# rainerzufalldererste/limg

Measured on AMD Instinct MI355X. Metric: encode Mpixels/s, 8K RGBA (limg_encode3d_test-equivalent: all 11 planes stored), higher is better.
Workload: dtype u8/i32 integer stage + f32 float stage (bit-exact vs the reference's strict SSE build)

## Files before the change

limg_amd/csrc/limg_hip_kernels.hip:

```cpp
#include "limg_hip_phase_e.h"
#include "limg_hip_lookback.h"

namespace limg_hip
{
  namespace
  {
    constexpr int kPrioE = 2;


    template <int CH, bool PERSIST, class P>
    __device__ __forceinline__ void finish_block(const P &p, const EStrip g, const uint32_t sb, const uint32_t bx, const BlkF *blkE, const uint32_t shift[3], const uint32_t fA,
                                                 const uint32_t fB, const uint32_t fC, const bool active, const uint32_t o, uint8_t *park, uint8_t *stage, uint32_t &waveCalls)
    {
      const uint32_t calls = (((shift[0] & 7u) + 7u) >> 3) + (((shift[1] & 7u) + 7u) >> 3) + (((shift[2] & 7u) + 7u) >> 3);
      waveCalls += calls;
      if (p.stripWords)
      {
        uint32_t words = 0;
#pragma unroll
        for (int k = 0; k < 3; k++)
        {
          const uint32_t sk = shift[k];
          if (sk < 8u) words += 8u - sk;
          else if (CH == 4 && sgpr((int)blkE->rec[8 * k + 3]) != sgpr((int)blkE->rec[8 * k + 7])) words += 8u;
// ... 37 lines not shown

    template <bool PERSIST, class P, class IO>
    __device__ __forceinline__ void park_or_store_factors(const P &p, const IO &io, const EStrip g, uint8_t *park, uint8_t *stage)
    {
      if (PERSIST)
        for (int i = g.tid; i < 384; i += kThreads) reinterpret_cast<uint4 *>(park + kParkFac)[i] = *reinterpret_cast<const uint4 *>(stage + (i >> 4) * kFacRow + (i & 15) * 16);
      else if (p.storePlanes) copy_factor_planes<true>(p, io, stage, g.x0, g.y0, g.stripW, g.ry, g.tid);
    }

    template <int CH, bool PERSIST, bool FAST, bool PREFIT, bool ACC, bool NOSEL, class P, class LIM, class IO>
    __device__ __forceinline__ void fit_search_strip(const P &p, const LIM &lim, const IO &io, const uint32_t id, const uint32_t local, const uint32_t rowBase, const uint32_t head0, uint8_t *lds,
                                                     uint8_t *park, const int tid)
    {
      constexpr LdsLayout LL = lds_layout<PREFIT>();
      EStrip g;
      g.tid = tid; g.lane = tid & 63; g.wave = tid >> 6;
      g.strip = local % p.stripsX; g.by = local / p.stripsX; g.byS = rowBase + g.by;
      g.x0 = g.strip * (kStripBlocks * kBlock); g.y0 = g.by * kBlock;
      g.stripW = min(p.sizeX - g.x0, (uint32_t)(kStripBlocks * kBlock)); g.ry = min(p.sizeY - g.y0, (uint32_t)kBlock);
      g.pix = reinterpret_cast<uint32_t *>(lds + kLdsStrip); g.V = reinterpret_cast<float *>(lds + LL.v); g.blk = reinterpret_cast<BlkF *>(lds + LL.blk);
      g.calls = reinterpret_cast<uint32_t *>(lds + LL.calls); g.trialc = reinterpret_cast<int *>(lds + LL.trialc);
      const int lane = g.lane;

      uint32_t recVal[2] = { 0u, 0u };
      if (PREFIT) request_prefit_records(p, g, recVal);
      stage_strip_pixels(p, io, g);
      __syncthreads();
      if (PREFIT) take_prefit_records<PERSIST>(p, g, recVal, park);
      else
      {
      const unsigned short *s_rsq = d_rsqrt_x86_tab;
      const int lane = g.lane, wave = g.wave;
      const uint32_t strip = g.strip, by = g.by, byS = g.byS;
      float *V = g.V + wave * kBatch * kVDw;
      BlkF *blk = g.blk + wave * kBlocksPerWave;
      auto geom = [&](int b, uint32_t &rx, uint32_t &n) -> bool { return block_geom(p, g, wave * kBlocksPerWave + b, rx, n); };

#pragma unroll 1
      for (int h = 0; h < kBlocksPerWave / kBatch; h++)
      {
      uint32_t px8[kBatch];
      V4 est8[kBatch];
      BlkF *const blkh = blk + h * kBatch;

#pragma unroll
      for (int i = 0; i < kBatch; i++)
      {
        const int b = h * kBatch + i;
        uint32_t rx, n;
        px8[i] = 0;
        est8[i].a = float2_t{ 0.0f, 0.0f }; est8[i].b = float2_t{ 0.0f, 0.0f };
        if (!geom(b, rx, n))
        {
// ... 161 lines not shown
        const int b = lane >> 3, j = lane & 7;
        const uint32_t flags = blk[b].flags;
        uint32_t big = 0;
#pragma unroll
        for (int r = 0; r < 3; r++)
        {
          const int kc = j + 8 * r, k = kc >> 2, c = kc & 3;
          const float *dir = r == 0 ? blk[b].dirA : (r == 1 ? blk[b].dirB : blk[b].dirC);
          const int sl = slot_of(c);
          float m = blk[b].mm[k], dv = dir[sl];
          const bool dead = (r == 2 && (flags & kZeroC)) || (r >= 1 && (flags & kZeroB)) || (flags & kZeroA);
          if (dead) { m = 0.0f; dv = 0.0f; }
          float val = m * dv;
          if (r == 0) val = blk[b].avg[sl] + val;
          int q = cvt_rne(val);
          if ((CH == 3 && c == 3) || !(flags & kValid)) q = 0;
          big |= (q > p.recordLimit || q < -p.recordLimit) ? 1u : 0u;
          blk[b].rec[kc] = (int16_t)q;
        }
        big |= (uint32_t)dpp<0xB1, 0xF>(0, (int)big);
        big |= (uint32_t)dpp<0x4E, 0xF>(0, (int)big);
        big |= (uint32_t)dpp<0x141, 0xF>(0, (int)big);
        if (j == 0 && big) blk[b].flags = flags | kBig;
      }
      wave_lds_fence();
      {
#pragma unroll
        for (int r = 0; r < 2; r++)
        {
          const int b = r * 4 + (lane >> 4), w = lane & 15;
          const uint32_t sb = wave * kBlocksPerWave + b, bx = strip * kStripBlocks + sb;
          const uint32_t val = w < 4 ? __float_as_uint(blk[b].avg[slot_of(w)]) : reinterpret_cast<const uint32_t *>(blk[b].rec)[w - 4];
          if (bx < p.blocksX && (!PERSIST || p.compactOut)) reinterpret_cast<uint32_t *>(p.records + (size_t)byS * p.blocksX + bx)[w] = val;
          if (PERSIST && w >= 4) reinterpret_cast<uint32_t *>(park + kParkRec)[sb * 12 + (w - 4)] = val;
        }
      }
    
      }
      if (!PERSIST && p.fitOnly) return;
      phase_e_view<CH, FAST, PREFIT>(g);
      uint32_t *s_queue = g.calls + 4;
      if (tid == 0) *s_queue = 0;
      __syncthreads();

      uint8_t *stage = reinterpret_cast<uint8_t *>(g.V);
      uint32_t waveCalls = 0;

      auto grab = [&]() -> uint32_t { uint32_t v = 0; if (lane == 0) v = atomicAdd(s_queue, 1u); return (uint32_t)sgpr((int)v); };
      uint32_t sbNext = grab();
#pragma unroll 1
      for (;;)
      {
        const uint32_t sb = sbNext;
        if (sb >= (uint32_t)kStripBlocks) break;
        uint32_t qv = 0;
        if (lane == 0) qv = atomicAdd(s_queue, 1u);
        uint32_t rx, n, lx, ly;
        if (!block_geom(p, g, sb, rx, n)) { sbNext = (uint32_t)sgpr((int)qv); continue; }
        const BlkF *const blkE = g.blk + sb;
        const bool active = (uint32_t)lane < n;
        const uint32_t px = block_pixel(g, sb, rx, n, lx, ly);
        uint32_t fA, fB, fC, shift[3] = { 0, 0, 0 };
        pixel_factors<CH, FAST>(reinterpret_cast<const BlkE *>(blkE), px, fA, fB, fC);
        if (p.forced[0] >= 0) { shift[0] = (uint32_t)p.forced[0]; shift[1] = (uint32_t)p.forced[1]; shift[2] = (uint32_t)p.forced[2]; }
        else if (lim.crushBits)
        {
// ... 79 lines not shown
        if (is_head(e)) { sum = 0; flag = 1; }
        sum += p.stripCalls[e];
      }
      s_sum[t] = sum; s_flag[t] = flag;
      __syncthreads();
      for (uint32_t off = 1; off < 1024; off <<= 1)
      {
        uint32_t vs = s_sum[t], vf = s_flag[t];
        if (t >= off && !vf) { vs += s_sum[t - off]; vf = s_flag[t - off]; }
        __syncthreads();
        s_sum[t] = vs; s_flag[t] = vf;
        __syncthreads();
      }
      uint32_t run = (t == 0) ? 0u : s_sum[t - 1];
      for (uint32_t e = begin; e < end; e++)
      {
        if (is_head(e)) run = 0;
        p.stripBase[e] = run;
        run += p.stripCalls[e];
      }
      if (p.chainCallsOut && end == total && begin < end) *p.chainCallsOut = run;
    }

    static_assert(kPhaseFBytes + kStripBlocks * 48 <= kLdsTotal - kLdsStrip - 16, "the F step's LDS overlays the E step's");

    template <int CH, bool PERSIST, class P, class IO>
    __device__ __forceinline__ void dither_store_strip(const P &p, const IO &io, const uint32_t id, const uint32_t local, const uint32_t rowBase, const uint32_t head0, uint8_t *fbase,
                                                       const uint8_t *park, const int tid)
    {
      int16_t *s_rec = reinterpret_cast<int16_t *>(fbase + kPhaseFBytes);
      const int lane = tid & 63, wave = tid >> 6;
      const uint32_t strip = local % p.stripsX, by = local / p.stripsX;
      const uint32_t byS = rowBase + by;
      const uint32_t x0 = strip * (kStripBlocks * kBlock), y0 = by * kBlock;
      const uint32_t stripW = min(p.sizeX - x0, (uint32_t)(kStripBlocks * kBlock));
      const uint32_t ry = min(p.sizeY - y0, (uint32_t)kBlock);
      const uint32_t nBlocks = min(p.blocksX - strip * kStripBlocks, (uint32_t)kStripBlocks);
      const StripLds L = carve_phase_f(fbase, s_rec, 24);

      if (PERSIST)
      {
        static_assert(kStripBlocks * 12 * 4 == 96 * 16, "record copy");
#pragma unroll 1
        for (int i = tid; i < 384; i += kThreads) *reinterpret_cast<uint4 *>(L.fac + (i >> 4) * kFacRow + (i & 15) * 16) = reinterpret_cast<const uint4 *>(park + kParkFac)[i];
        if (tid < 96) reinterpret_cast<uint4 *>(s_rec)[tid] = reinterpret_cast<const uint4 *>(park + kParkRec)[tid];
        if (tid < kStripBlocks) L.shift[tid] = (uint32_t)tid < nBlocks ? reinterpret_cast<const uint32_t *>(park + kParkShift)[tid] : 0u;
      }
      else
      {
        copy_factor_planes<false>(p, io, L.fac, x0, y0, stripW, ry, tid);
        for (int i = tid; i < kStripBlocks * 12; i += kThreads)
        {
          const int sb = i / 12, w = i - sb * 12;
          uint32_t v = 0;
          if ((uint32_t)sb < nBlocks) v = reinterpret_cast<const uint32_t *>(p.records + (size_t)byS * p.blocksX + strip * kStripBlocks + sb)[4 + w];
          reinterpret_cast<uint32_t *>(s_rec + sb * 24)[w] = v;
        }
        if (tid < kStripBlocks) L.shift[tid] = (uint32_t)tid < nBlocks ? p.shifts[(size_t)byS * p.blocksX + strip * kStripBlocks + tid] : 0u;
      }
      __syncthreads();
      phase_f_prepare<CH>(L, lane, wave, p.recordLimit);
      wave_lds_fence();
      const bool rowsPath = PERSIST || (p.sizeX % kBlock == 0 && ry == (uint32_t)kBlock);
      if (p.fullPlanes) phase_f_store_const(p, io, L, x0, y0, ry, lane, wave, rowsPath ? 1u : 3u);
      if (wave == 0)
      {
        uint32_t base;
        if (PERSIST)
        {
          const uint32_t headId = head0 + chain_head_row(p.chainCount, p.chainRows, by) * p.stripsX;
          const uint32_t w = lane < kStripBlocks ? L.shift[lane] : 0u;
          const uint32_t agg = wave_sum(w >> 24);
          const unsigned long long own = desc_load(p.desc + id);
          if ((uint32_t)(own >> 32) == kDescInclusive) base = (uint32_t)sgpr((int)((uint32_t)own == kBasePoison ? kBasePoison : (uint32_t)own - agg));
          else
          {
            base = lookback_base(p, id, headId, agg, lane);
            if (lane == 0 && publishes(p, id)) desc_store(p.desc + id, kDescInclusive, base == kBasePoison ? kBasePoison : base + agg);
          }
#ifdef LIMG_HIP_TEST_HOOKS
          if (id == p.testBaseErrStrip) base += 1u;
#endif
        }
        else
        {
          base = p.stripBase[id];
          if (p.chainBase) base += (uint32_t)*p.chainBase;
        }
        phase_f_first_calls(L, base, lane);
      }
      __syncthreads();
      if (PERSIST && L.first[0] == kBasePoison) return;
      if (rowsPath) phase_f_rows<CH>(p, io, L, strip, x0, y0, lane, wave, [&]() { if (p.fullPlanes) phase_f_store_const(p, io, L, x0, y0, ry, lane, wave, 2u); });
      else phase_f_pixels<CH>(p, io, L, strip, x0, y0, ry, lane, wave, tid);
    }

    template <int CH, bool FAST, bool PREFIT, bool ACC>
    __global__ __launch_bounds__(kThreads) void k_fit_search(const EncodeParams p)
    {
      __shared__ __attribute__((aligned(16))) uint8_t s_lds[lds_layout<PREFIT>().total];
      if (red_select_dead(p.maxPixel32)) fit_search_strip<CH, false, FAST, PREFIT, ACC, true>(p, p, p.io, blockIdx.x, blockIdx.x, 0u, 0u, s_lds, nullptr, (int)threadIdx.x);
      else fit_search_strip<CH, false, FAST, PREFIT, ACC, false>(p, p, p.io, blockIdx.x, blockIdx.x, 0u, 0u, s_lds, nullptr, (int)threadIdx.x);
    }

    template <int CH>
    __global__ __launch_bounds__(kThreads) void k_dither_store(const EncodeParams p)
    {
      __shared__ __attribute__((aligned(16))) uint8_t s_lds[kPhaseFBytes + kStripBlocks * 48];
      if (p.chainBase && *p.chainBase == ~0ull) return;
      dither_store_strip<CH, false>(p, p.io, blockIdx.x, blockIdx.x, 0u, 0u, s_lds, nullptr, (int)threadIdx.x);
    }

    template <int CH, bool FAST, bool PREFIT, bool ACC>
    __global__ __launch_bounds__(kThreads, PREFIT ? 6 : 5) void k_encode_persistent(const EncodeParams p)
    {
      __shared__ __attribute__((aligned(16))) uint8_t s_lds[lds_layout<PREFIT>().total];
      __shared__ uint32_t s_ticket;
      typedef const __attribute__((address_space(4))) EncodeParams KernArgs;
      typedef const __attribute__((address_space(4))) ImageIO KernIO;
      auto io_of = [](KernArgs *a, uint32_t img) -> KernIO * { return a->batchCount > 1 ? (KernIO *)a->batch + img : &a->io; };
#define LIMG_LOOP_LIMITS(a, img) (*(a))
#define LIMG_LOOP_STRIPS (p.imageStrips * p.batchCount)
#define LIMG_LOOP_FIND_IMAGE(a, t, img) if ((a)->batchCount > 1) img = (t) / (a)->imageStrips;
#define LIMG_LOOP_HEAD0(a, img) ((img) * (a)->imageStrips)
#define LIMG_LOOP_ROWBASE(a, img) ((img) * (a)->blocksY)
#define LIMG_LOOP_VIEW(a, img) (a)
      if (red_select_dead(p.maxPixel32))
      {
        constexpr bool NOSEL = true;
#include "limg_hip_persistent_loop.inc"
      }
// ... 190 lines not shown
```

limg_amd/csrc/limg_hip_phase_e.h:

```cpp
#ifndef LIMG_HIP_PHASE_E_H
#define LIMG_HIP_PHASE_E_H

#include "limg_hip_search.h"
#include "limg_hip_phase_f.h"
#include "limg_hip_float_pixel.h"

namespace limg_hip
{
  namespace
  {
    constexpr int kLdsStrip = 0, kLdsV = kLdsStrip + 8 * kRowDw * 4, kLdsVBytes = kWaves * kBatch * kVDw * 4;
    constexpr int kLdsBlk = kLdsV + kLdsVBytes, kLdsCalls = kLdsBlk + kStripBlocks * 192, kLdsTotal = kLdsCalls + 32;
    static_assert(kLdsTotal <= 32768 - 16, "5 workgroups per CU");
    struct LdsLayout { int v, blk, calls, trialc, total; };
    constexpr int kTrialConstDw = 20;
    template <bool PREFIT> __device__ __host__ constexpr LdsLayout lds_layout()
    {
      if (!PREFIT) return LdsLayout{ kLdsV, kLdsBlk, kLdsCalls, kLdsV, kLdsTotal };
      const int v = kLdsStrip + 8 * kRowDw * 4, blk = v + kFacBytes, calls = blk + kStripBlocks * 192, tc = calls + 32, e = tc + kStripBlocks * kTrialConstDw * 4;
      const int f = kLdsStrip + kPhaseFBytes + kStripBlocks * 48 + 16;
      return LdsLayout{ v, blk, calls, tc, e > f ? e : f };
    }
    static_assert(lds_layout<true>().total <= 163840 / 6, "6 workgroups per CU with the float stage in its own kernel");


    constexpr int kParkFac = 0, kParkRec = 6144, kParkShift = 6144 + 1536, kParkBytes = 8192;


    template <class P>
    __device__ __forceinline__ void request_prefit_records(const P &p, const EStrip g, uint32_t recVal[2])
    {
#pragma unroll
      for (int r = 0; r < 2; r++)
      {
        const int b = r * 4 + (g.lane >> 4), w = g.lane & 15;
        const uint32_t bx = g.strip * kStripBlocks + g.wave * kBlocksPerWave + b;
        if (bx < p.blocksX) recVal[r] = w >= 4 ? reinterpret_cast<const uint32_t *>(p.records + (size_t)g.byS * p.blocksX + bx)[w]
                                               : reinterpret_cast<const uint32_t *>(p.invN)[((size_t)g.byS * p.blocksX + bx) * 4 + w];
      }
    }

    template <class P, class IO>
    __device__ __forceinline__ void stage_strip_pixels(const P &p, const IO &io, const EStrip g)
    {
      const int tid = g.tid;
      if (p.vecIn)
      {
#pragma unroll
        for (int pass = 0; pass < 2; pass++)
        {
          const uint32_t row = pass * 4 + (tid >> 6), col = (tid & 63) * 4;
          if (row < g.ry && col < g.stripW)
          {
            const uint4 v = *reinterpret_cast<const uint4 *>(io.in + (size_t)(g.y0 + row) * p.sizeX + g.x0 + col);
            *reinterpret_cast<uint4 *>(&g.pix[row * kRowDw + col]) = v;
          }
        }
      }
      else
      {
        for (uint32_t i = tid; i < 8 * 256; i += kThreads)
        {
          const uint32_t row = i >> 8, col = i & 255;
          if (row < g.ry && col < g.stripW) g.pix[row * kRowDw + col] = io.in[(size_t)(g.y0 + row) * p.sizeX + g.x0 + col];
        }
      }
    }

    template <bool PERSIST, class P>
    __device__ __forceinline__ void take_prefit_records(const P &p, const EStrip g, const uint32_t recVal[2], uint8_t *park)
    {
      BlkF *blk = g.blk + g.wave * kBlocksPerWave;
#pragma unroll
      for (int r = 0; r < 2; r++)
      {
        const int b = r * 4 + (g.lane >> 4), w = g.lane & 15;
        const uint32_t sb = g.wave * kBlocksPerWave + b, bx = g.strip * kStripBlocks + sb;
        const uint32_t val = recVal[r];
        if (w < 3) reinterpret_cast<BlkE *>(&blk[b])->invN[w] = __uint_as_float(val);
        if (w >= 4)
        {
          reinterpret_cast<uint32_t *>(blk[b].rec)[w - 4] = val;
          if (PERSIST) reinterpret_cast<uint32_t *>(park + kParkRec)[sb * 12 + (w - 4)] = val;
        }
        const int lo = (int)(int16_t)(val & 0xFFFFu), hi = (int)(int16_t)(val >> 16);
        uint32_t big = (w >= 4 && (lo > p.recordLimit || lo < -p.recordLimit || hi > p.recordLimit || hi < -p.recordLimit)) ? 1u : 0u;
        big |= (uint32_t)dpp<0xB1, 0xF>(0, (int)big);
        big |= (uint32_t)dpp<0x4E, 0xF>(0, (int)big);
        big |= (uint32_t)dpp<0x141, 0xF>(0, (int)big);
        big |= (uint32_t)dpp<0x140, 0xF>(0, (int)big);
        if (w == 0) { blk[b].flags = (bx < p.blocksX ? kValid : 0u) | (big ? kBig : 0u); blk[b].n = bx < p.blocksX ? 64u : 0u; }
      }
      wave_lds_fence();
    }

    template <int CH, bool FAST, bool PREFIT>
    __device__ __forceinline__ void phase_e_view(const EStrip g)
    {
      const int lane = g.lane;
      BlkF *blk = g.blk + g.wave * kBlocksPerWave;
      float nrm[2], off[2], invn[2];
#pragma unroll
      for (int r = 0; r < 2; r++)
      {
        const int idx = min(r * 64 + lane, 95);
        const int b = idx / 12, fc = idx - b * 12, f = fc >> 2, c = fc & 3;
        const int lo = blk[b].rec[f * 8 + c], hi = blk[b].rec[f * 8 + 4 + c];
        nrm[r] = (float)(hi - lo); off[r] = (float)lo;
        if (PREFIT) { invn[r] = 0.0f; continue; }
        const float sq = nrm[r] * nrm[r];
        const float s0 = __int_as_float(dpp<0x00, 0xF>(0, __float_as_int(sq))), s1 = __int_as_float(dpp<0x55, 0xF>(0, __float_as_int(sq)));
        const float s2 = __int_as_float(dpp<0xAA, 0xF>(0, __float_as_int(sq))), s3 = __int_as_float(dpp<0xFF, 0xF>(0, __float_as_int(sq)));
        float s = ((0.0f + s0) + s1) + s2;
        if (CH == 4) s = s + s3;
        const bool nz = (s0 != 0.0f) || (s1 != 0.0f) || (s2 != 0.0f) || (CH == 4 && s3 != 0.0f);
        invn[r] = nz ? (FAST ? __builtin_amdgcn_rcpf(s) : 1.0f / s) : 0.0f;
      }
      wave_lds_fence();
#pragma unroll
      for (int r = 0; r < 2; r++)
      {
        const int idx = r * 64 + lane;
        if (idx < 96)
        {
          const int b = idx / 12, fc = idx - b * 12, f = fc >> 2, c = fc & 3;
          BlkE *e = reinterpret_cast<BlkE *>(&blk[b]);
          e->nrm[f][slot_of(c)] = nrm[r]; e->off[f][slot_of(c)] = off[r];
          if (!PREFIT && c == 0) e->invN[f] = invn[r];
          if (PREFIT && c < 3)
          {
            int *tc = g.trialc + (g.wave * kBlocksPerWave + b) * kTrialConstDw;
            tc[f * 3 + c] = -(int)nrm[r];
            tc[9 + f * 3 + c] = term_const(f, c, (int)off[r]);
          }
        }
      }
    }

    template <int CH, bool FAST>
    __device__ __forceinline__ void pixel_factors(const BlkE *be, const uint32_t px, uint32_t &fA, uint32_t &fB, uint32_t &fC)
    {
      const V4 pv = px_to_v4(px);
      const V4 nA = ld4(be->nrm[0]), mnA = ld4(be->off[0]);
      const float fa = dp4<CH, FAST>(pv - mnA, nA) * be->invN[0];
      fA = cvt_u8_rne_sat(255.0f * fa);
      const V4 nB = ld4(be->nrm[1]), ofB = ld4(be->off[1]);
      V4 est = mnA + nA * fa;
      const float fb = dp4<CH, FAST>((pv - est) - ofB, nB) * be->invN[1];
      fB = cvt_u8_rne_sat(255.0f * fb);
      const V4 nC = ld4(be->nrm[2]), ofC = ld4(be->off[2]);
      est = est + nB * fb;
      const float fc = dp4<CH, FAST>((pv - est) - ofC, nC) * be->invN[2];
      fC = cvt_u8_rne_sat(255.0f * fc);
    }
  }
}

// ... 2 lines not shown
```

limg_amd/csrc/limg_hip_phase_f.h:

```cpp
#ifndef LIMG_HIP_PHASE_F_H
#define LIMG_HIP_PHASE_F_H

#include "limg_hip_search.h"
#include <type_traits>

namespace limg_hip
{
  namespace
  {
    constexpr int kFacRow = 320, kFacPlane = 8 * kFacRow, kFacBytes = 3 * kFacPlane;

    template <bool TO_PLANES, class P, class IO>
    __device__ __forceinline__ void copy_factor_planes(const P &p, const IO &io, uint8_t *fac, const uint32_t x0, const uint32_t y0, const uint32_t stripW, const uint32_t ry, const int tid)
    {
      uint8_t *planes[3] = { io.info.pFactorsA, io.info.pFactorsB, io.info.pFactorsC };
      auto piece = [&](auto *g, auto *l) { if (TO_PLANES) *g = *l; else *l = *g; };
      if (p.vecFactors)
        for (int i = tid; i < 384; i += kThreads)
        {
          const int pl = i >> 7, row = (i & 127) >> 4, col = (i & 15) * 16;
          if ((uint32_t)row < ry && (uint32_t)col < stripW)
            piece(reinterpret_cast<uint4 *>(planes[pl] + (size_t)(y0 + row) * p.sizeX + x0 + col), reinterpret_cast<uint4 *>(fac + pl * kFacPlane + row * kFacRow + col));
        }
      else
        for (int i = tid; i < 3 * 2048; i += kThreads)
        {
          const int pl = i >> 11, row = (i & 2047) >> 8, col = i & 255;
          if ((uint32_t)row < ry && (uint32_t)col < stripW) piece(planes[pl] + (size_t)(y0 + row) * p.sizeX + x0 + col, fac + pl * kFacPlane + row * kFacRow + col);
        }
    }

    struct StripLds
    {
      uint8_t *fac;
      uint32_t *dec;
      uint8_t *out;
      uint32_t *cst;
      int32_t *nm;
      uint32_t *shift;
      uint32_t *first;
      uint32_t *flags;
      const int16_t *rec;
      int recStride;
    };
    constexpr int kPhaseFBytes = kFacBytes + 8192 + 3584 + 3072 + 128 + 128 + 128;

    __device__ __forceinline__ StripLds carve_phase_f(uint8_t *base, const int16_t *rec, int recStride)
    {
      StripLds L;
      L.fac = base;
      L.dec = reinterpret_cast<uint32_t *>(base + kFacBytes);
      L.out = base;
      L.cst = reinterpret_cast<uint32_t *>(base + kFacBytes + 8192);
      L.nm = reinterpret_cast<int32_t *>(base + kFacBytes + 8192 + 3584);
      L.shift = reinterpret_cast<uint32_t *>(base + kFacBytes + 8192 + 3584 + 3072);
      L.first = L.shift + 32;
      L.flags = L.shift + 64;
      L.rec = rec; L.recStride = recStride;
      return L;
    }

    __device__ __forceinline__ constexpr int decode_bias(int factor, int c) { return c < 2 ? (term_bias(factor) << 8) : 0; }

    template <int CH>
    __device__ __forceinline__ void phase_f_prepare(const StripLds &L, int lane, int wave, int recordLimit)
    {
      if (lane < 56)
      {
        const int b = lane / 7, k = lane - b * 7, sb = wave * kBlocksPerWave + b;
        const int16_t *rec = L.rec + sb * L.recStride;
        uint32_t v;
        if (k == 0)
        {
          const uint32_t w = L.shift[sb];
          const uint32_t pat[3] = { (w & 0xFF), ((w >> 8) & 0xFF), ((w >> 16) & 0xFF) };
          const uint32_t pa = pat[0] == 8 ? 0xFFu : pat[0] * 0x22u, pb = pat[1] == 8 ? 0xFFu : pat[1] * 0x22u, pc = pat[2] == 8 ? 0xFFu : pat[2] * 0x22u;
          v = 0xFF000000u | (pa << 16) | (pb << 8) | pc;
        }
        else
        {
          v = 0;
#pragma unroll
          for (int c = 0; c < CH; c++)
          {
            int q = rec[(k - 1) * 4 + c] + (k >= 3 ? 0x80 : 0);
            q = q < 0 ? 0 : (q > 255 ? 255 : q);
            v |= (uint32_t)q << (8 * c);
          }
          if (CH == 3) v |= 0xFF000000u;
        }
        reinterpret_cast<uint4 *>(L.cst)[k * kStripBlocks + sb] = make_uint4(v, v, v, v);
      }
      if (lane < kBlocksPerWave)
      {
        const int sb = wave * kBlocksPerWave + lane;
        const int16_t *rec = L.rec + sb * L.recStride;
        uint32_t fl;
        if (CH == 3) fl = 255u << 8;
        else
        {
          const bool varies = rec[7] != rec[3] || rec[15] != rec[11] || rec[23] != rec[19];
          int a = rec[3] + rec[11] + rec[19];
          a = a < 0 ? 0 : (a > 255 ? 255 : a);
          fl = varies ? 2u : ((uint32_t)a << 8);
        }
        L.flags[sb] = fl;
      }
      wave_lds_fence();
#pragma unroll
      for (int r = 0; r < 2; r++)
      {
        const int idx = r * 64 + lane;
        if (idx < 96)
        {
          const int b = idx / 12, fc = idx - b * 12, f = fc >> 2, c = fc & 3, sb = wave * kBlocksPerWave + b;
          const int16_t *rec = L.rec + sb * L.recStride;
          const uint32_t sh = (L.shift[sb] >> (8 * f)) & 0xFF;
          const int lo = rec[f * 8 + c], hi = rec[f * 8 + 4 + c];
          if ((uint32_t)(lo + recordLimit) > 2u * (uint32_t)recordLimit || (uint32_t)(hi + recordLimit) > 2u * (uint32_t)recordLimit) atomicOr(&L.flags[sb], 1u);
          int n = hi - lo, m = lo;
          if (c < 3)
          {
            if (sh > 7) { n = 0; if (f > 0) m = 0; }
          }
          else if (CH == 3) { n = 0; m = 0xFFFF; }
          int *dst = L.nm + sb * 24;
          dst[f * 4 + c] = n;
          dst[12 + f * 4 + c] = (int)(((uint32_t)m << 8) + 128u + (uint32_t)(c < 2 ? (f == 2 ? 0x200000 : 0x300000) : 0));
        }
      }
    }

    typedef uint32_t u32x4_t __attribute__((ext_vector_type(4)));
    typedef uint32_t u32x2_t __attribute__((ext_vector_type(2)));
    __device__ __forceinline__ void plane_store16(void *dst, const uint4 &v)
    {
      __builtin_nontemporal_store(u32x4_t{ v.x, v.y, v.z, v.w }, reinterpret_cast<u32x4_t *>(dst));
    }
    __device__ __forceinline__ void plane_store8(void *dst, const uint2 &v)
    {
      __builtin_nontemporal_store(u32x2_t{ v.x, v.y }, reinterpret_cast<u32x2_t *>(dst));
    }

    template <class P, class IO>
    __device__ __forceinline__ void phase_f_store_const(const P &p, const IO &io, const StripLds &L, uint32_t x0, uint32_t y0, uint32_t ry, int lane, int wave, const uint32_t halves = 3u)
    {
      const uint32_t wx0 = x0 + wave * 64;
      if (wx0 >= p.sizeX) return;
      const uint32_t ww = min(p.sizeX - wx0, 64u);
      uint32_t *planes[7] = { io.info.pShiftABCX, io.info.pColAMin, io.info.pColAMax, io.info.pColBMin, io.info.pColBMax, io.info.pColCMin, io.info.pColCMax };
      if (p.vecPlanes)
      {
        const uint32_t col = ((uint32_t)lane & 15u) * 4u, rsub = (uint32_t)lane >> 4;
// ... 87 lines not shown
      const uint32_t j = (uint32_t)lane & 7u, r = (uint32_t)lane >> 3;
      const uint32_t sb = (uint32_t)wave * kBlocksPerWave + j, bx = strip * kStripBlocks + sb;
      const bool valid = bx < p.blocksX;
      const uint32_t w = L.shift[sb], fl = L.flags[sb];
      uint32_t call = L.first[sb];
      const size_t g = (size_t)(y0 + r) * p.sizeX + x0 + sb * kBlock;
      uint2 nz[3];
#pragma unroll
      for (int k = 0; k < 3; k++)
      {
        const uint32_t s = (w >> (8 * k)) & 0xFFu;
        nz[k] = make_uint2(0u, 0u);
        if (((s - 1u) < 7u) && valid)
        {
          nz[k] = *reinterpret_cast<const uint2 *>(p.noise + (size_t)min(call, p.noiseLast) * 64 + r * 8);
          call++;
        }
      }
      between();
      const uint8_t *facRow = L.fac + r * kFacRow + sb * kBlock;
      const int *nm = L.nm + sb * 24;
      const bool generic = __builtin_amdgcn_ballot_w64((fl & 1u) != 0u) != 0ull;
      const bool anyAlpha = CH == 4 && __builtin_amdgcn_ballot_w64((fl & 2u) != 0u) != 0ull;
      const bool rawEscape = !p.fullPlanes && p.streamRaw;
      auto consts = [&](int k, uint32_t &negHalf, uint32_t &shr, uint32_t &mul, uint32_t &keep, uint2 &fq, uint2 &nzm)
      {
        const uint32_t s = (w >> (8 * k)) & 0xFFu;
        shr = (((s - 1u) < 7u) && valid) ? s : 0u;
        negHalf = 0u - ((1u << shr) >> 1);
        mul = (1u << s) + __builtin_amdgcn_perm(0x7F150401u, 0u, s);
        keep = (0xFFu << s) & 0xFFu;
        if (rawEscape && s == 8) keep = 0xFFu;
        fq = *reinterpret_cast<const uint2 *>(facRow + k * kFacPlane);
        const uint32_t m4 = __builtin_amdgcn_perm(0u, (1u << shr) - 1u, 0u);
        nzm = make_uint2(nz[k].x & m4, nz[k].y & m4);
      };
      uint8_t *planes8[3] = { io.info.pFactorsA, io.info.pFactorsB, io.info.pFactorsC };
      auto store_factor = [&](int k, uint32_t lo, uint32_t hi)
      {
        if (!valid) return;
        if (p.vecFactors8) plane_store8(planes8[k] + g, make_uint2(lo, hi));
        else
        {
#pragma unroll
          for (int i = 0; i < 4; i++) { planes8[k][g + i] = (uint8_t)(lo >> (8 * i)); planes8[k][g + 4 + i] = (uint8_t)(hi >> (8 * i)); }
        }
      };
      uint32_t px[8];
      if (!generic)
      {
        uint32_t accRG[8], lo, hi, negHalf, shr, mul, keep;
        int accB[8], accA[8];
        uint2 fq, nzm;
#define LIMG_ROWS_FACTOR(K, ALPHA)                                                                                                                         \
        consts(K, negHalf, shr, mul, keep, fq, nzm);                                                                                                      \
        rows_factor<K, ALPHA>(fq, nzm, negHalf, shr, mul, keep, *reinterpret_cast<const int4 *>(nm + 4 * K), *reinterpret_cast<const int4 *>(nm + 12 + 4 * K), accRG, accB, accA, lo, hi); \
        store_factor(K, lo, hi);                                                                                                                          \
// ... 195 lines not shown
```

limg_amd/csrc/limg_hip_rate.hip:

```cpp
#include "limg_hip_phase_e.h"

namespace limg_hip
{
  namespace
  {
    __device__ __forceinline__ void set_thresholds(RateDevice *d, uint32_t errorFactor)
    {
      const Thresholds t = thresholds(errorFactor);
      d->maxPixel32 = t.maxPixel32; d->blockLimitFull = t.blockLimitFull; d->maxBlock = t.maxBlock; d->crushBits = t.crushBits;
    }

    __global__ void k_rate_begin(RateDevice *d, unsigned long long *counter, const RateState first, const uint32_t firstErrorFactor)
    {
      d->search = first;
      d->listNext = 0u;
      set_thresholds(d, firstErrorFactor);
      *counter = 0ull;
    }

    __global__ void k_rate_step(RateDevice *d, unsigned long long *counter, const unsigned long long fixedBytes, const uint32_t *list, unsigned long long *listBytes,
                                const uint32_t listCount)
    {
      const unsigned long long bytes = fixedBytes + 8ull * *counter;
      *counter = 0ull;
// ... 8 lines not shown
      }
      if (d->search.done) return;
      rate_step(d->search, bytes);
      if (!d->search.done) set_thresholds(d, 2u * d->search.next);
    }

    template <int CH, bool FAST, class P, class IO>
    __device__ __forceinline__ void rate_probe_strip(const P &p, const IO &io, const RateDevice *const st, unsigned long long *const counter, uint8_t *const lds,
                                                     const uint32_t strip, const uint32_t by, const uint32_t byS)
    {
      constexpr LdsLayout LL = lds_layout<true>();
      if (st->search.done) return;
      const uint32_t maxPixel32 = (uint32_t)sgpr((int)st->maxPixel32), blockLimit = (uint32_t)sgpr((int)st->blockLimitFull), crushBits = (uint32_t)sgpr((int)st->crushBits);
      const int tid = (int)threadIdx.x;
      EStrip g;
      g.tid = tid; g.lane = tid & 63; g.wave = tid >> 6;
      g.strip = strip; g.by = by; g.byS = byS;
      g.x0 = g.strip * (kStripBlocks * kBlock); g.y0 = g.by * kBlock;
      g.stripW = min(p.sizeX - g.x0, (uint32_t)(kStripBlocks * kBlock)); g.ry = (uint32_t)kBlock;
      g.pix = reinterpret_cast<uint32_t *>(lds + kLdsStrip); g.V = reinterpret_cast<float *>(lds + LL.v); g.blk = reinterpret_cast<BlkF *>(lds + LL.blk);
      g.calls = reinterpret_cast<uint32_t *>(lds + LL.calls); g.trialc = reinterpret_cast<int *>(lds + LL.trialc);
      const int lane = g.lane;

      uint32_t recVal[2] = { 0u, 0u };
      request_prefit_records(p, g, recVal);
      stage_strip_pixels(p, io, g);
      __syncthreads();
      take_prefit_records<false>(p, g, recVal, nullptr);
      phase_e_view<CH, FAST, true>(g);
      uint32_t *s_queue = g.calls + 4;
      if (tid == 0) *s_queue = 0;
      __syncthreads();

      uint32_t waveWords = 0;
      auto grab = [&]() -> uint32_t { uint32_t v = 0; if (lane == 0) v = atomicAdd(s_queue, 1u); return (uint32_t)sgpr((int)v); };
      uint32_t sbNext = grab();
#pragma unroll 1
      for (;;)
      {
        const uint32_t sb = sbNext;
        if (sb >= (uint32_t)kStripBlocks) break;
        uint32_t qv = 0;
        if (lane == 0) qv = atomicAdd(s_queue, 1u);
        uint32_t rx, n, lx, ly;
        if (!block_geom(p, g, sb, rx, n)) { sbNext = (uint32_t)sgpr((int)qv); continue; }
        const BlkF *const blkE = g.blk + sb;
        uint32_t shift[3] = { 0, 0, 0 };
        if (p.forced[0] >= 0) { shift[0] = (uint32_t)p.forced[0]; shift[1] = (uint32_t)p.forced[1]; shift[2] = (uint32_t)p.forced[2]; }
        else if (crushBits)
        {
          const uint32_t px = block_pixel(g, sb, rx, n, lx, ly);
          uint32_t fA, fB, fC;
          pixel_factors<CH, FAST>(reinterpret_cast<const BlkE *>(blkE), px, fA, fB, fC);
// ... 119 lines not shown
```

limg_amd/csrc/limg_hip_search.h:

```cpp
#ifndef LIMG_HIP_SEARCH_H
#define LIMG_HIP_SEARCH_H

#include "limg_hip_device.h"
#include "limg_search_table.h"

namespace limg_hip
{
  namespace
  {
    struct __attribute__((aligned(32))) SearchEntry { uint32_t w[8]; };
    __constant__ SearchEntry d_search_tab[LIMG_SEARCH_STATES] = LIMG_SEARCH_TABLE_INIT;

    typedef short short2_t __attribute__((ext_vector_type(2)));
    typedef unsigned short ushort2_t __attribute__((ext_vector_type(2)));
    __device__ __forceinline__ constexpr int term_bias(int factor) { return factor == 2 ? 0x2000 : 0x3000; }
    __device__ __forceinline__ int term_const(int f, int c, int lo) { return 255 - ((lo << 8) + 128) + (c < 2 ? (term_bias(f) << 8) : 0); }

    struct TrialState
    {
      uint32_t fA, fB, fC;
      uint32_t loRG, hiRG;
      int pxB, pxBlo;
      int nA[3], nB[3], nC[3];
      int mA[3], mB[3], mC[3];
      uint32_t tA_RG, tB_RG, tC_RG;
      int tA_B, tB_B, tC_B;
      uint32_t cA, cB, cC;
    };

    __device__ __forceinline__ void make_terms(const uint32_t f, const uint32_t s, const uint32_t mul, const int n[3], const int m[3], uint32_t &tRG, int &tB)
    {
      const int d = (int)mul_u24_uniform(f >> (s & 31u), mul);
      const int t0 = mad_i24(d, n[0], m[0]), t1 = mad_i24(d, n[1], m[1]), t2 = mad_i24(d, n[2], m[2]);
      tRG = __builtin_amdgcn_perm((uint32_t)t1, (uint32_t)t0, 0x06050201u);
      tB = t2 >> 8;
    }

    __device__ __forceinline__ void rebuild_A(TrialState &t, const uint32_t sA, const uint32_t mul) { make_terms(t.fA, sA, mul, t.nA, t.mA, t.tA_RG, t.tA_B); t.cA = sA; }
    __device__ __forceinline__ void rebuild_B(TrialState &t, const uint32_t sB, const uint32_t mul)
// ... 177 lines not shown
```

Baseline: 56920.

## Build per-block record constants in one wave overlapped with pixel staging

Per-block record and invN loading plus derivation of E-step constants (nrm/off/trial terms) now run on a single dedicated wave, one lane per block, overlapping the strip pixel staging and removing a barrier and the separate phase_e_view pass on the prefit path. The F-step prepare similarly moves to one wave that reads records from registers, with per-shift constants precomputed into a small LDS table instead of computed per call, and the big-record flag parked. This cuts barriers and redundant LDS round-trips but serialises constant setup onto fewer lanes, adds an LDS table and changes LDS layout.

```diff
diff --git a/limg_amd/csrc/limg_hip_kernels.hip b/limg_amd/csrc/limg_hip_kernels.hip
--- a/limg_amd/csrc/limg_hip_kernels.hip
+++ b/limg_amd/csrc/limg_hip_kernels.hip
@@ -83,13 +83,21 @@
       g.calls = reinterpret_cast<uint32_t *>(lds + LL.calls); g.trialc = reinterpret_cast<int *>(lds + LL.trialc);
       const int lane = g.lane;
 
-      uint32_t recVal[2] = { 0u, 0u };
-      if (PREFIT) request_prefit_records(p, g, recVal);
+      uint32_t *s_queue = g.calls + 4;
+      if (PREFIT)
+      {
+        BlockRecord rec;
+        const bool recordWave = sgpr(g.wave) == kRecordWave;
+        if (recordWave) request_prefit_records(p, g, rec);
+        stage_strip_pixels(p, io, g);
+        if (recordWave) block_constants_e<PERSIST>(p, g, rec, park);
+        if (tid == 0) *s_queue = 0;
+        __syncthreads();
+      }
+      else
+      {
       stage_strip_pixels(p, io, g);
       __syncthreads();
-      if (PREFIT) take_prefit_records<PERSIST>(p, g, recVal, park);
-      else
-      {
       const unsigned short *s_rsq = d_rsqrt_x86_tab;
       const int lane = g.lane, wave = g.wave;
       const uint32_t strip = g.strip, by = g.by, byS = g.byS;
@@ -297,6 +305,7 @@
         big |= (uint32_t)dpp<0x4E, 0xF>(0, (int)big);
         big |= (uint32_t)dpp<0x141, 0xF>(0, (int)big);
         if (j == 0 && big) blk[b].flags = flags | kBig;
+        if (PERSIST && j == 0) reinterpret_cast<uint32_t *>(park + kParkFlag)[wave * kBlocksPerWave + b] = big;
       }
       wave_lds_fence();
       {
@@ -313,10 +322,12 @@
     
       }
       if (!PERSIST && p.fitOnly) return;
-      phase_e_view<CH, FAST, PREFIT>(g);
-      uint32_t *s_queue = g.calls + 4;
-      if (tid == 0) *s_queue = 0;
-      __syncthreads();
+      if (!PREFIT)
+      {
+        phase_e_view<CH, FAST>(g);
+        if (tid == 0) *s_queue = 0;
+        __syncthreads();
+      }
 
       uint8_t *stage = reinterpret_cast<uint8_t *>(g.V);
       uint32_t waveCalls = 0;
@@ -442,13 +453,12 @@
       if (p.chainCallsOut && end == total && begin < end) *p.chainCallsOut = run;
     }
 
-    static_assert(kPhaseFBytes + kStripBlocks * 48 <= kLdsTotal - kLdsStrip - 16, "the F step's LDS overlays the E step's");
+    static_assert(kPhaseFBytes <= kLdsTotal - kLdsStrip - 16, "the F step's LDS overlays the E step's");
 
     template <int CH, bool PERSIST, class P, class IO>
     __device__ __forceinline__ void dither_store_strip(const P &p, const IO &io, const uint32_t id, const uint32_t local, const uint32_t rowBase, const uint32_t head0, uint8_t *fbase,
                                                        const uint8_t *park, const int tid)
     {
-      int16_t *s_rec = reinterpret_cast<int16_t *>(fbase + kPhaseFBytes);
       const int lane = tid & 63, wave = tid >> 6;
       const uint32_t strip = local % p.stripsX, by = local / p.stripsX;
       const uint32_t byS = rowBase + by;
@@ -456,31 +466,42 @@
       const uint32_t stripW = min(p.sizeX - x0, (uint32_t)(kStripBlocks * kBlock));
       const uint32_t ry = min(p.sizeY - y0, (uint32_t)kBlock);
       const uint32_t nBlocks = min(p.blocksX - strip * kStripBlocks, (uint32_t)kStripBlocks);
-      const StripLds L = carve_phase_f(fbase, s_rec, 24);
-
+      const StripLds L = carve_phase_f(fbase);
+
+      uint4 rec[3];
+      uint32_t shiftWord, bigFlag;
+      const bool prepareWave = sgpr(wave) == kPrepareWave;
+      const bool prepares = prepareWave && (uint32_t)lane < nBlocks;
+      if (prepareWave)
+      {
+        rec[0] = rec[1] = rec[2] = make_uint4(0u, 0u, 0u, 0u); shiftWord = 0u; bigFlag = 0u;
+        if (prepares)
+        {
+          if (PERSIST)
+          {
+            const uint4 *src = reinterpret_cast<const uint4 *>(park + kParkRec) + lane * 3;
+            rec[0] = src[0]; rec[1] = src[1]; rec[2] = src[2];
+            bigFlag = reinterpret_cast<const uint32_t *>(park + kParkFlag)[lane];
+            shiftWord = reinterpret_cast<const uint32_t *>(park + kParkShift)[lane];
+          }
+          else
+          {
+            const size_t bi = (size_t)byS * p.blocksX + strip * kStripBlocks + lane;
+            const uint32_t *src = reinterpret_cast<const uint32_t *>(p.records + bi) + 4;
+#pragma unroll
+            for (int i = 0; i < 3; i++) rec[i] = make_uint4(src[4 * i], src[4 * i + 1], src[4 * i + 2], src[4 * i + 3]);
+            shiftWord = p.shifts[bi];
+          }
+        }
+      }
       if (PERSIST)
       {
-        static_assert(kStripBlocks * 12 * 4 == 96 * 16, "record copy");
 #pragma unroll 1
         for (int i = tid; i < 384; i += kThreads) *reinterpret_cast<uint4 *>(L.fac + (i >> 4) * kFacRow + (i & 15) * 16) = reinterpret_cast<const uint4 *>(park + kParkFac)[i];
-        if (tid < 96) reinterpret_cast<uint4 *>(s_rec)[tid] = reinterpret_cast<const uint4 *>(park + kParkRec)[tid];
-        if (tid < kStripBlocks) L.shift[tid] = (uint32_t)tid < nBlocks ? reinterpret_cast<const uint32_t *>(park + kParkShift)[tid] : 0u;
-      }
-      else
-      {
-        copy_factor_planes<false>(p, io, L.fac, x0, y0, stripW, ry, tid);
-        for (int i = tid; i < kStripBlocks * 12; i += kThreads)
-        {
-          const int sb = i / 12, w = i - sb * 12;
-          uint32_t v = 0;
-          if ((uint32_t)sb < nBlocks) v = reinterpret_cast<const uint32_t *>(p.records + (size_t)byS * p.blocksX + strip * kStripBlocks + sb)[4 + w];
-          reinterpret_cast<uint32_t *>(s_rec + sb * 24)[w] = v;
-        }
-        if (tid < kStripBlocks) L.shift[tid] = (uint32_t)tid < nBlocks ? p.shifts[(size_t)byS * p.blocksX + strip * kStripBlocks + tid] : 0u;
-      }
+      }
+      else copy_factor_planes<false>(p, io, L.fac, x0, y0, stripW, ry, tid);
+      if (prepareWave) phase_f_prepare<CH, PERSIST>(L, lane, prepares, rec, shiftWord, bigFlag, p.recordLimit, !p.fullPlanes && p.streamRaw);
       __syncthreads();
-      phase_f_prepare<CH>(L, lane, wave, p.recordLimit);
-      wave_lds_fence();
       const bool rowsPath = PERSIST || (p.sizeX % kBlock == 0 && ry == (uint32_t)kBlock);
       if (p.fullPlanes) phase_f_store_const(p, io, L, x0, y0, ry, lane, wave, rowsPath ? 1u : 3u);
       if (wave == 0)
@@ -526,7 +547,7 @@
     template <int CH>
     __global__ __launch_bounds__(kThreads) void k_dither_store(const EncodeParams p)
     {
-      __shared__ __attribute__((aligned(16))) uint8_t s_lds[kPhaseFBytes + kStripBlocks * 48];
+      __shared__ __attribute__((aligned(16))) uint8_t s_lds[kPhaseFBytes];
       if (p.chainBase && *p.chainBase == ~0ull) return;
       dither_store_strip<CH, false>(p, p.io, blockIdx.x, blockIdx.x, 0u, 0u, s_lds, nullptr, (int)threadIdx.x);
     }
diff --git a/limg_amd/csrc/limg_hip_phase_e.h b/limg_amd/csrc/limg_hip_phase_e.h
--- a/limg_amd/csrc/limg_hip_phase_e.h
+++ b/limg_amd/csrc/limg_hip_phase_e.h
@@ -18,25 +18,28 @@
     {
       if (!PREFIT) return LdsLayout{ kLdsV, kLdsBlk, kLdsCalls, kLdsV, kLdsTotal };
       const int v = kLdsStrip + 8 * kRowDw * 4, blk = v + kFacBytes, calls = blk + kStripBlocks * 192, tc = calls + 32, e = tc + kStripBlocks * kTrialConstDw * 4;
-      const int f = kLdsStrip + kPhaseFBytes + kStripBlocks * 48 + 16;
+      const int f = kLdsStrip + kPhaseFBytes + 16;
       return LdsLayout{ v, blk, calls, tc, e > f ? e : f };
     }
     static_assert(lds_layout<true>().total <= 163840 / 6, "6 workgroups per CU with the float stage in its own kernel");
 
 
-    constexpr int kParkFac = 0, kParkRec = 6144, kParkShift = 6144 + 1536, kParkBytes = 8192;
+    constexpr int kParkFac = 0, kParkRec = 6144, kParkShift = 6144 + 1536, kParkFlag = kParkShift + 128, kParkBytes = 8192;
+    static_assert(kParkFlag + 128 <= kParkBytes, "park slot");
 
 
+    constexpr int kRecordWave = kWaves - 1;
+    struct BlockRecord { uint4 rec[3], invN; };
     template <class P>
-    __device__ __forceinline__ void request_prefit_records(const P &p, const EStrip g, uint32_t recVal[2])
+    __device__ __forceinline__ void request_prefit_records(const P &p, const EStrip g, BlockRecord &r)
     {
-#pragma unroll
-      for (int r = 0; r < 2; r++)
+      const uint32_t bx = g.strip * kStripBlocks + (uint32_t)g.lane;
+      if (g.lane < kStripBlocks && bx < p.blocksX)
       {
-        const int b = r * 4 + (g.lane >> 4), w = g.lane & 15;
-        const uint32_t bx = g.strip * kStripBlocks + g.wave * kBlocksPerWave + b;
-        if (bx < p.blocksX) recVal[r] = w >= 4 ? reinterpret_cast<const uint32_t *>(p.records + (size_t)g.byS * p.blocksX + bx)[w]
-                                               : reinterpret_cast<const uint32_t *>(p.invN)[((size_t)g.byS * p.blocksX + bx) * 4 + w];
+        const size_t bi = (size_t)g.byS * p.blocksX + bx;
+        const uint4 *src = reinterpret_cast<const uint4 *>(p.records + bi);
+        r.rec[0] = src[1]; r.rec[1] = src[2]; r.rec[2] = src[3];
+        r.invN = reinterpret_cast<const uint4 *>(p.invN)[bi];
       }
     }
 
@@ -68,33 +71,51 @@
     }
 
     template <bool PERSIST, class P>
-    __device__ __forceinline__ void take_prefit_records(const P &p, const EStrip g, const uint32_t recVal[2], uint8_t *park)
+    __device__ __forceinline__ void block_constants_e(const P &p, const EStrip g, const BlockRecord &r, uint8_t *park)
     {
-      BlkF *blk = g.blk + g.wave * kBlocksPerWave;
+      if (g.lane >= kStripBlocks) return;
+      const uint32_t sb = (uint32_t)g.lane;
+      BlkF *blk = g.blk + sb;
+      if (g.strip * kStripBlocks + sb >= p.blocksX)
+      {
+        *reinterpret_cast<uint2 *>(&blk->flags) = make_uint2(0u, 0u);
+        return;
+      }
+      const bool big = record_beyond_limit(r.rec, p.recordLimit);
+      BlkE *e = reinterpret_cast<BlkE *>(blk);
+      int *tc = g.trialc + sb * kTrialConstDw;
+      int n[3][3], m[3][3];
 #pragma unroll
-      for (int r = 0; r < 2; r++)
+      for (int f = 0; f < 3; f++)
       {
-        const int b = r * 4 + (g.lane >> 4), w = g.lane & 15;
-        const uint32_t sb = g.wave * kBlocksPerWave + b, bx = g.strip * kStripBlocks + sb;
-        const uint32_t val = recVal[r];
-        if (w < 3) reinterpret_cast<BlkE *>(&blk[b])->invN[w] = __uint_as_float(val);
-        if (w >= 4)
-        {
-          reinterpret_cast<uint32_t *>(blk[b].rec)[w - 4] = val;
-          if (PERSIST) reinterpret_cast<uint32_t *>(park + kParkRec)[sb * 12 + (w - 4)] = val;
-        }
-        const int lo = (int)(int16_t)(val & 0xFFFFu), hi = (int)(int16_t)(val >> 16);
-        uint32_t big = (w >= 4 && (lo > p.recordLimit || lo < -p.recordLimit || hi > p.recordLimit || hi < -p.recordLimit)) ? 1u : 0u;
-        big |= (uint32_t)dpp<0xB1, 0xF>(0, (int)big);
-        big |= (uint32_t)dpp<0x4E, 0xF>(0, (int)big);
-        big |= (uint32_t)dpp<0x141, 0xF>(0, (int)big);
-        big |= (uint32_t)dpp<0x140, 0xF>(0, (int)big);
-        if (w == 0) { blk[b].flags = (bx < p.blocksX ? kValid : 0u) | (big ? kBig : 0u); blk[b].n = bx < p.blocksX ? 64u : 0u; }
+        const uint4 q = r.rec[f];
+        const int lo[4] = { (int)(int16_t)(q.x & 0xFFFFu), (int)q.x >> 16, (int)(int16_t)(q.y & 0xFFFFu), (int)q.y >> 16 };
+        const int hi[4] = { (int)(int16_t)(q.z & 0xFFFFu), (int)q.z >> 16, (int)(int16_t)(q.w & 0xFFFFu), (int)q.w >> 16 };
+        *reinterpret_cast<float4 *>(e->nrm[f]) = make_float4((float)(hi[0] - lo[0]), (float)(hi[2] - lo[2]), (float)(hi[1] - lo[1]), (float)(hi[3] - lo[3]));
+        *reinterpret_cast<float4 *>(e->off[f]) = make_float4((float)lo[0], (float)lo[2], (float)lo[1], (float)lo[3]);
+#pragma unroll
+        for (int c = 0; c < 3; c++) { n[f][c] = lo[c] - hi[c]; m[f][c] = term_const(f, c, lo[c]); }
       }
-      wave_lds_fence();
+      static_assert(offsetof(BlkE, invN) % 16 == 0 && sizeof(BlkE) <= 112 && offsetof(BlkF, flags) == 120 && offsetof(BlkF, rec) == 128 && kTrialConstDw % 4 == 0, "16-byte stores");
+      *reinterpret_cast<uint4 *>(e->invN) = r.invN;
+      *reinterpret_cast<uint2 *>(&blk->flags) = make_uint2(kValid | (big ? kBig : 0u), 64u);
+      uint4 *rec = reinterpret_cast<uint4 *>(blk->rec);
+      rec[0] = r.rec[0]; rec[1] = r.rec[1]; rec[2] = r.rec[2];
+      int4 *tc4 = reinterpret_cast<int4 *>(tc);
+      tc4[0] = make_int4(n[0][0], n[0][1], n[0][2], n[1][0]);
+      tc4[1] = make_int4(n[1][1], n[1][2], n[2][0], n[2][1]);
+      tc4[2] = make_int4(n[2][2], m[0][0], m[0][1], m[0][2]);
+      tc4[3] = make_int4(m[1][0], m[1][1], m[1][2], m[2][0]);
+      *reinterpret_cast<int2 *>(tc + 16) = make_int2(m[2][1], m[2][2]);
+      if (PERSIST)
+      {
+        uint4 *prec = reinterpret_cast<uint4 *>(park + kParkRec) + sb * 3;
+        prec[0] = r.rec[0]; prec[1] = r.rec[1]; prec[2] = r.rec[2];
+        reinterpret_cast<uint32_t *>(park + kParkFlag)[sb] = big ? 1u : 0u;
+      }
     }
 
-    template <int CH, bool FAST, bool PREFIT>
+    template <int CH, bool FAST>
     __device__ __forceinline__ void phase_e_view(const EStrip g)
     {
       const int lane = g.lane;
@@ -107,7 +128,6 @@
         const int b = idx / 12, fc = idx - b * 12, f = fc >> 2, c = fc & 3;
         const int lo = blk[b].rec[f * 8 + c], hi = blk[b].rec[f * 8 + 4 + c];
         nrm[r] = (float)(hi - lo); off[r] = (float)lo;
-        if (PREFIT) { invn[r] = 0.0f; continue; }
         const float sq = nrm[r] * nrm[r];
         const float s0 = __int_as_float(dpp<0x00, 0xF>(0, __float_as_int(sq))), s1 = __int_as_float(dpp<0x55, 0xF>(0, __float_as_int(sq)));
         const float s2 = __int_as_float(dpp<0xAA, 0xF>(0, __float_as_int(sq))), s3 = __int_as_float(dpp<0xFF, 0xF>(0, __float_as_int(sq)));
@@ -126,13 +146,7 @@
           const int b = idx / 12, fc = idx - b * 12, f = fc >> 2, c = fc & 3;
           BlkE *e = reinterpret_cast<BlkE *>(&blk[b]);
           e->nrm[f][slot_of(c)] = nrm[r]; e->off[f][slot_of(c)] = off[r];
-          if (!PREFIT && c == 0) e->invN[f] = invn[r];
-          if (PREFIT && c < 3)
-          {
-            int *tc = g.trialc + (g.wave * kBlocksPerWave + b) * kTrialConstDw;
-            tc[f * 3 + c] = -(int)nrm[r];
-            tc[9 + f * 3 + c] = term_const(f, c, (int)off[r]);
-          }
+          if (c == 0) e->invN[f] = invn[r];
         }
       }
     }
diff --git a/limg_amd/csrc/limg_hip_phase_f.h b/limg_amd/csrc/limg_hip_phase_f.h
--- a/limg_amd/csrc/limg_hip_phase_f.h
+++ b/limg_amd/csrc/limg_hip_phase_f.h
@@ -40,12 +40,12 @@
       uint32_t *shift;
       uint32_t *first;
       uint32_t *flags;
-      const int16_t *rec;
-      int recStride;
+      uint32_t *tab;
     };
-    constexpr int kPhaseFBytes = kFacBytes + 8192 + 3584 + 3072 + 128 + 128 + 128;
-
-    __device__ __forceinline__ StripLds carve_phase_f(uint8_t *base, const int16_t *rec, int recStride)
+    constexpr int kShiftTabDw = 8;
+    constexpr int kPhaseFBytes = kFacBytes + 8192 + 3584 + 3072 + 128 + 128 + 128 + 9 * kShiftTabDw * 4;
+
+    __device__ __forceinline__ StripLds carve_phase_f(uint8_t *base)
     {
       StripLds L;
       L.fac = base;
@@ -56,79 +56,88 @@
       L.shift = reinterpret_cast<uint32_t *>(base + kFacBytes + 8192 + 3584 + 3072);
       L.first = L.shift + 32;
       L.flags = L.shift + 64;
-      L.rec = rec; L.recStride = recStride;
+      L.tab = L.shift + 96;
       return L;
     }
 
     __device__ __forceinline__ constexpr int decode_bias(int factor, int c) { return c < 2 ? (term_bias(factor) << 8) : 0; }
 
-    template <int CH>
-    __device__ __forceinline__ void phase_f_prepare(const StripLds &L, int lane, int wave, int recordLimit)
-    {
-      if (lane < 56)
-      {
-        const int b = lane / 7, k = lane - b * 7, sb = wave * kBlocksPerWave + b;
-        const int16_t *rec = L.rec + sb * L.recStride;
-        uint32_t v;
-        if (k == 0)
-        {
-          const uint32_t w = L.shift[sb];
-          const uint32_t pat[3] = { (w & 0xFF), ((w >> 8) & 0xFF), ((w >> 16) & 0xFF) };
-          const uint32_t pa = pat[0] == 8 ? 0xFFu : pat[0] * 0x22u, pb = pat[1] == 8 ? 0xFFu : pat[1] * 0x22u, pc = pat[2] == 8 ? 0xFFu : pat[2] * 0x22u;
-          v = 0xFF000000u | (pa << 16) | (pb << 8) | pc;
-        }
-        else
-        {
-          v = 0;
-#pragma unroll
-          for (int c = 0; c < CH; c++)
-          {
-            int q = rec[(k - 1) * 4 + c] + (k >= 3 ? 0x80 : 0);
-            q = q < 0 ? 0 : (q > 255 ? 255 : q);
-            v |= (uint32_t)q << (8 * c);
-          }
-          if (CH == 3) v |= 0xFF000000u;
-        }
-        reinterpret_cast<uint4 *>(L.cst)[k * kStripBlocks + sb] = make_uint4(v, v, v, v);
-      }
-      if (lane < kBlocksPerWave)
-      {
-        const int sb = wave * kBlocksPerWave + lane;
-        const int16_t *rec = L.rec + sb * L.recStride;
-        uint32_t fl;
-        if (CH == 3) fl = 255u << 8;
-        else
-        {
-          const bool varies = rec[7] != rec[3] || rec[15] != rec[11] || rec[23] != rec[19];
-          int a = rec[3] + rec[11] + rec[19];
-          a = a < 0 ? 0 : (a > 255 ? 255 : a);
-          fl = varies ? 2u : ((uint32_t)a << 8);
-        }
-        L.flags[sb] = fl;
-      }
-      wave_lds_fence();
-#pragma unroll
-      for (int r = 0; r < 2; r++)
-      {
-        const int idx = r * 64 + lane;
-        if (idx < 96)
-        {
-          const int b = idx / 12, fc = idx - b * 12, f = fc >> 2, c = fc & 3, sb = wave * kBlocksPerWave + b;
-          const int16_t *rec = L.rec + sb * L.recStride;
-          const uint32_t sh = (L.shift[sb] >> (8 * f)) & 0xFF;
-          const int lo = rec[f * 8 + c], hi = rec[f * 8 + 4 + c];
-          if ((uint32_t)(lo + recordLimit) > 2u * (uint32_t)recordLimit || (uint32_t)(hi + recordLimit) > 2u * (uint32_t)recordLimit) atomicOr(&L.flags[sb], 1u);
-          int n = hi - lo, m = lo;
-          if (c < 3)
-          {
-            if (sh > 7) { n = 0; if (f > 0) m = 0; }
-          }
-          else if (CH == 3) { n = 0; m = 0xFFFF; }
-          int *dst = L.nm + sb * 24;
-          dst[f * 4 + c] = n;
-          dst[12 + f * 4 + c] = (int)(((uint32_t)m << 8) + 128u + (uint32_t)(c < 2 ? (f == 2 ? 0x200000 : 0x300000) : 0));
-        }
-      }
+    constexpr int kPrepareWave = 1;
+    template <int CH, bool PARKED>
+    __device__ __forceinline__ void phase_f_prepare(const StripLds &L, const int lane, const bool exists, const uint4 rec[3], const uint32_t w, const uint32_t parkedFlag, const int recordLimit,
+                                                    const bool rawEscape)
+    {
+      if (lane >= kStripBlocks)
+      {
+        const uint32_t s = (uint32_t)lane - kStripBlocks;
+        if (s > 8u) return;
+        const uint32_t shr = (s - 1u) < 7u ? s : 0u, mask = (1u << shr) - 1u;
+        const uint32_t keep = (rawEscape && s == 8u) ? 0xFFu : ((0xFFu << s) & 0xFFu);
+        *reinterpret_cast<uint4 *>(L.tab + s * kShiftTabDw) = make_uint4(0u - ((1u << shr) >> 1), shr, shift_mul(s), keep);
+        L.tab[s * kShiftTabDw + 4] = mask * 0x01010101u;
+        return;
+      }
+      const int sb = lane;
+      if (!exists)
+      {
+        L.shift[sb] = 0u; L.flags[sb] = 0u;
+        return;
+      }
+      L.shift[sb] = w;
+      const bool big = PARKED ? parkedFlag != 0u : record_beyond_limit(rec, recordLimit);
+      uint4 *cst = reinterpret_cast<uint4 *>(L.cst) + sb;
+      {
+        const uint32_t t = w & 0xFFFFFFu;
+        const uint32_t v = mul_u24(t, 0x22u) - mul_u24((t >> 3) & 0x010101u, 0x11u);
+        const uint32_t pat = __builtin_amdgcn_perm(v, v, 0x0D000102u);
+        cst[0] = make_uint4(pat, pat, pat, pat);
+      }
+      const uint32_t d[12] = { rec[0].x, rec[0].y, rec[0].z, rec[0].w, rec[1].x, rec[1].y, rec[1].z, rec[1].w, rec[2].x, rec[2].y, rec[2].z, rec[2].w };
+#pragma unroll
+      for (int k = 1; k < 7; k++)
+      {
+        short2_t a = __builtin_bit_cast(short2_t, d[2 * (k - 1)]), b = __builtin_bit_cast(short2_t, d[2 * (k - 1) + 1]);
+        if (k >= 3)
+        {
+          a = __builtin_elementwise_add_sat(a, short2_t{ 0x80, 0x80 });
+          b = __builtin_elementwise_add_sat(b, short2_t{ 0x80, 0x80 });
+        }
+        a = __builtin_elementwise_min(__builtin_elementwise_max(a, short2_t{ 0, 0 }), short2_t{ 255, 255 });
+        b = __builtin_elementwise_min(__builtin_elementwise_max(b, short2_t{ 0, 0 }), short2_t{ 255, 255 });
+        const uint32_t v = __builtin_amdgcn_perm(__builtin_bit_cast(uint32_t, b), __builtin_bit_cast(uint32_t, a), CH == 3 ? 0x0D040200u : 0x06040200u);
+        cst[k * kStripBlocks] = make_uint4(v, v, v, v);
+      }
+      int4 *nm = reinterpret_cast<int4 *>(L.nm + sb * 24);
+      int loA[3], hiA[3];
+#pragma unroll
+      for (int f = 0; f < 3; f++)
+      {
+        const uint4 q = rec[f];
+        const int lo[4] = { (int)(int16_t)(q.x & 0xFFFFu), (int)q.x >> 16, (int)(int16_t)(q.y & 0xFFFFu), (int)q.y >> 16 };
+        const int hi[4] = { (int)(int16_t)(q.z & 0xFFFFu), (int)q.z >> 16, (int)(int16_t)(q.w & 0xFFFFu), (int)q.w >> 16 };
+        const bool zero = ((w >> (8 * f)) & 0xFFu) > 7u;
+        int n[4], m[4];
+#pragma unroll
+        for (int c = 0; c < 4; c++)
+        {
+          n[c] = hi[c] - lo[c]; m[c] = lo[c];
+          if (c < 3) { if (zero) { n[c] = 0; if (f > 0) m[c] = 0; } }
+          else if (CH == 3) { n[c] = 0; m[c] = 0xFFFF; }
+          m[c] = (int)(((uint32_t)m[c] << 8) + 128u + (uint32_t)decode_bias(f, c));
+        }
+        nm[f] = make_int4(n[0], n[1], n[2], n[3]);
+        nm[3 + f] = make_int4(m[0], m[1], m[2], m[3]);
+        loA[f] = lo[3]; hiA[f] = hi[3];
+      }
+      uint32_t fl;
+      if (CH == 3) fl = 255u << 8;
+      else
+      {
+        const bool varies = hiA[0] != loA[0] || hiA[1] != loA[1] || hiA[2] != loA[2];
+        const int a = med3_i32(loA[0] + loA[1] + loA[2], 0, 255);
+        fl = varies ? 2u : ((uint32_t)a << 8);
+      }
+      L.flags[sb] = fl | (big ? 1u : 0u);
     }
 
     typedef uint32_t u32x4_t __attribute__((ext_vector_type(4)));
@@ -262,17 +271,13 @@
       const int *nm = L.nm + sb * 24;
       const bool generic = __builtin_amdgcn_ballot_w64((fl & 1u) != 0u) != 0ull;
       const bool anyAlpha = CH == 4 && __builtin_amdgcn_ballot_w64((fl & 2u) != 0u) != 0ull;
-      const bool rawEscape = !p.fullPlanes && p.streamRaw;
       auto consts = [&](int k, uint32_t &negHalf, uint32_t &shr, uint32_t &mul, uint32_t &keep, uint2 &fq, uint2 &nzm)
       {
-        const uint32_t s = (w >> (8 * k)) & 0xFFu;
-        shr = (((s - 1u) < 7u) && valid) ? s : 0u;
-        negHalf = 0u - ((1u << shr) >> 1);
-        mul = (1u << s) + __builtin_amdgcn_perm(0x7F150401u, 0u, s);
-        keep = (0xFFu << s) & 0xFFu;
-        if (rawEscape && s == 8) keep = 0xFFu;
+        const uint32_t *e = L.tab + ((w >> (8 * k)) & 0xFFu) * kShiftTabDw;
+        const uint4 t = *reinterpret_cast<const uint4 *>(e);
+        negHalf = t.x; shr = t.y; mul = t.z; keep = t.w;
+        const uint32_t m4 = e[4];
         fq = *reinterpret_cast<const uint2 *>(facRow + k * kFacPlane);
-        const uint32_t m4 = __builtin_amdgcn_perm(0u, (1u << shr) - 1u, 0u);
         nzm = make_uint2(nz[k].x & m4, nz[k].y & m4);
       };
       uint8_t *planes8[3] = { io.info.pFactorsA, io.info.pFactorsB, io.info.pFactorsC };
diff --git a/limg_amd/csrc/limg_hip_rate.hip b/limg_amd/csrc/limg_hip_rate.hip
--- a/limg_amd/csrc/limg_hip_rate.hip
+++ b/limg_amd/csrc/limg_hip_rate.hip
@@ -54,13 +54,12 @@
       g.calls = reinterpret_cast<uint32_t *>(lds + LL.calls); g.trialc = reinterpret_cast<int *>(lds + LL.trialc);
       const int lane = g.lane;
 
-      uint32_t recVal[2] = { 0u, 0u };
-      request_prefit_records(p, g, recVal);
+      uint32_t *s_queue = g.calls + 4;
+      BlockRecord rec;
+      const bool recordWave = sgpr(g.wave) == kRecordWave;
+      if (recordWave) request_prefit_records(p, g, rec);
       stage_strip_pixels(p, io, g);
-      __syncthreads();
-      take_prefit_records<false>(p, g, recVal, nullptr);
-      phase_e_view<CH, FAST, true>(g);
-      uint32_t *s_queue = g.calls + 4;
+      if (recordWave) block_constants_e<false>(p, g, rec, nullptr);
       if (tid == 0) *s_queue = 0;
       __syncthreads();
 
diff --git a/limg_amd/csrc/limg_hip_search.h b/limg_amd/csrc/limg_hip_search.h
--- a/limg_amd/csrc/limg_hip_search.h
+++ b/limg_amd/csrc/limg_hip_search.h
@@ -15,6 +15,18 @@
     typedef unsigned short ushort2_t __attribute__((ext_vector_type(2)));
     __device__ __forceinline__ constexpr int term_bias(int factor) { return factor == 2 ? 0x2000 : 0x3000; }
     __device__ __forceinline__ int term_const(int f, int c, int lo) { return 255 - ((lo << 8) + 128) + (c < 2 ? (term_bias(f) << 8) : 0); }
+    __device__ __forceinline__ bool record_beyond_limit(const uint4 rec[3], const int limit)
+    {
+      const uint32_t d[12] = { rec[0].x, rec[0].y, rec[0].z, rec[0].w, rec[1].x, rec[1].y, rec[1].z, rec[1].w, rec[2].x, rec[2].y, rec[2].z, rec[2].w };
+      short2_t mn = __builtin_bit_cast(short2_t, d[0]), mx = mn;
+#pragma unroll
+      for (int i = 1; i < 12; i++)
+      {
+        mn = __builtin_elementwise_min(mn, __builtin_bit_cast(short2_t, d[i]));
+        mx = __builtin_elementwise_max(mx, __builtin_bit_cast(short2_t, d[i]));
+      }
+      return max((int)mx.x, (int)mx.y) > limit || min((int)mn.x, (int)mn.y) < -limit;
+    }
 
     struct TrialState
     {
```

New measurement: 57170, median of 6. Within noise of the previous version (+0.4%).
